# lzhangbj/deep_video_interpolation_extrapolation

Measured on AMD Instinct MI355X. Metric: train frames/s (256x512 len-3 clips), higher is better.
Workload: dtype bf16; 1 GPU; InterNet int_5_len_3 train step 256x512 bf16; per_gpu_batch=8, global_batch=8, parallelism=dp1, step=eager, executor side-stream lanes

## Files before the change

deep_video_interpolation_extrapolation_amd/_lib.py:

```python
import ctypes
import os
import threading

import torch

LIB_PATH = os.path.join(os.path.dirname(os.path.abspath(__file__)), "libdvie.so")

DVIE_OK = 0
DVIE_EINVAL = 1001
F32, BF16 = 0, 1
ACT_NONE, ACT_LRELU, ACT_ELU, ACT_RELU, ACT_TANH = 0, 1, 2, 3, 4
EW_FUSE, EW_UPT, EW_POOL, EW_POOLT, EW_COPY, EW_L1SIGN, EW_NCHW, EW_TONCHW, EW_MASK, EW_IM2COL, EW_LABELS = range(11)
LOSS_L1, LOSS_GDL, LOSS_SSIM, LOSS_MSE, LOSS_CE, LOSS_L1NHWC, LOSS_COSNHWC, LOSS_IOU, LOSS_ARGMAX_IOU = range(9)
OP_CONV, OP_WGRAD, OP_WREDUCE, OP_COLSUM, OP_EW, OP_LOSS, OP_PACK = 1, 2, 3, 4, 5, 6, 7
OP_BN_FWD, OP_BN_BWD, OP_HEAD_FWD, OP_HEAD_BWD, OP_ATTN, OP_HEAD3_BWD, OP_SEGENC_FWD = 8, 9, 10, 11, 12, 13, 14
OP_SEGENC_BWD = 15
OP_WREDUCE_MULTI = 16
OP_COSFEAT = 17
COSFEAT_MAX_TAPS = 8
YUV_420, YUV_444 = 420, 444
(ATTN_L2NORM, ATTN_L2NORM_BWD, ATTN_CORR, ATTN_GATHER, ATTN_GATHER_T, ATTN_SOFTMAX, ATTN_SOFTMAX_BWD, ATTN_WNORM,
 ATTN_WNORM_BWD, ATTN_POOL, ATTN_POOL_T) = range(11)

vp = ctypes.c_void_p
# ... 283 lines not shown
        ("n", i32), ("h", i32), ("w", i32), ("kpad0", i32), ("kpad2", i32), ("kpad4", i32),
    ]


class SegencBwdDesc(ctypes.Structure):
    _fields_ = [
        ("dout", vp), ("e2", vp), ("e1", vp), ("inp", vp), ("w4d", vp), ("w2d", vp),
        ("dw4", vp), ("dw2", vp), ("dw0", vp), ("db4", vp), ("db2", vp), ("db0", vp),
        ("dout_ld", i64), ("e2_ld", i64), ("e1_ld", i64), ("in_ld", i64),
        ("n", i32), ("h", i32), ("w", i32), ("kpad4", i32), ("kpad2", i32), ("slabs", i32),
    ]


class WreduceMultiDesc(ctypes.Structure):
    _fields_ = [("descs", vp), ("n", i32), ("pad", i32)]


class _OpUnion(ctypes.Union):
    _fields_ = [
        ("conv", ConvDesc), ("wgrad", WgradDesc), ("wreduce", WreduceDesc), ("colsum", ColsumDesc),
        ("ew", EwDesc), ("loss", LossDesc), ("pack", PackList), ("bn", BnDesc), ("head", HeadDesc),
        ("attn", AttnDesc), ("head3", Head3BwdDesc), ("segenc", SegencDesc), ("segenc_bwd", SegencBwdDesc),
        ("wreduce_multi", WreduceMultiDesc), ("cosfeat", CosFeatDesc),
    ]


class Op(ctypes.Structure):
    _fields_ = [("kind", i32), ("lane", i32), ("u", _OpUnion)]


_ABI = {0: Op, OP_CONV: ConvDesc, OP_WGRAD: WgradDesc, OP_WREDUCE: WreduceDesc, OP_COLSUM: ColsumDesc,
        OP_EW: EwDesc, OP_LOSS: LossDesc, OP_PACK: PackDesc, OP_BN_FWD: BnDesc, OP_HEAD_FWD: HeadDesc,
        OP_ATTN: AttnDesc, OP_HEAD3_BWD: Head3BwdDesc, OP_SEGENC_FWD: SegencDesc, OP_SEGENC_BWD: SegencBwdDesc, OP_WREDUCE_MULTI: WreduceMultiDesc,
        OP_COSFEAT: CosFeatDesc, 100: WarpDesc, 101: SoftmaxDesc, 102: SnLayer, 103: ClipDesc,
        104: SynthLoadDesc, 105: SynthFinishDesc, 106: SynthBridgeDesc, 107: SynthScoreDesc,
        108: SynthLoadPadDesc, 109: SynthFinishCropDesc, 110: SynthVggLoadDesc}
_ABI_MORE = {111: SynthMsssimDesc, 112: SynthYuvDesc, 113: SynthSceneDesc, 114: SynthCutFillDesc,
             115: SynthTileBlendDesc, 117: SynthRetimeDesc}

EXPORTS = [
    "dvie_conv2d_fwd", "dvie_conv2d_wgrad", "dvie_wgrad_splits_hint", "dvie_wgrad_slabs", "dvie_wgrad_reduce", "dvie_wgrad_reduce_multi", "dvie_colsum", "dvie_pack_weights",
    "dvie_ew", "dvie_loss", "dvie_loss_partial_count", "dvie_loss_ws_floats", "dvie_warp_fwd",
    "dvie_warp_bwd", "dvie_adamax", "dvie_scale", "dvie_run_ops", "dvie_abi_sizeof", "dvie_version",
    "dvie_last_error", "dvie_bn_fwd", "dvie_bn_bwd", "dvie_bn_partial_splits", "dvie_head_fwd", "dvie_head_bwd",
    "dvie_softmax_fwd", "dvie_softmax_bwd", "dvie_adam", "dvie_sn_fwd", "dvie_sn_bwd", "dvie_reparam_fwd",
    "dvie_reparam_bwd", "dvie_warp_ws_floats", "dvie_clip_prep", "dvie_attn", "dvie_step_inc", "dvie_adamax_dev",
    "dvie_adam_dev", "dvie_mfma_probe", "dvie_launch_probe", "dvie_sum_f32", "dvie_wgrad_bias_slabs", "dvie_head3_bwd",
    "dvie_segenc_fwd", "dvie_segenc_bwd", "dvie_pack_blocks", "dvie_trace_kernels", "dvie_traced_kernels",
    "dvie_synth_load", "dvie_synth_finish", "dvie_synth_bridge", "dvie_synth_score", "dvie_synth_score_ws_bytes",
    "dvie_synth_load_pad", "dvie_synth_finish_crop", "dvie_conv_zbits", "dvie_bn_partial_doubles",
    "dvie_synth_vgg_load", "dvie_cosfeat", "dvie_cosfeat_blocks", "dvie_synth_msssim", "dvie_synth_msssim_ws_bytes",
    "dvie_synth_yuv2rgb", "dvie_synth_rgb2yuv", "dvie_conv_chain", "dvie_conv2d_chain", "dvie_ops_chain_pairs",
    "dvie_synth_scene", "dvie_synth_scene_ws_bytes", "dvie_synth_cutfill", "dvie_synth_tile_blend",
    "dvie_synth_retime",
]

_lib = None
_lock = threading.Lock()


class DvieError(RuntimeError):
    pass


def load():
    global _lib
    if _lib is not None:
        return _lib
    with _lock:
        if _lib is not None:
            return _lib
        if not os.path.exists(LIB_PATH):
            raise DvieError(
                f"{LIB_PATH} is missing: build it with `python -c 'import __graft_entry__ as g; g.build()'` "
                "(there is no non-HIP fallback)")
        lib = ctypes.CDLL(LIB_PATH)
        lib.dvie_abi_sizeof.restype = ctypes.c_size_t
        lib.dvie_abi_sizeof.argtypes = [i32]
        for which, st in {**_ABI, **_ABI_MORE}.items():
            got = lib.dvie_abi_sizeof(which)
            if got != ctypes.sizeof(st):
                raise DvieError(f"ABI mismatch for {st.__name__}: C {got} vs ctypes {ctypes.sizeof(st)}")
        lib.dvie_version.restype = ctypes.c_char_p
        lib.dvie_last_error.restype = ctypes.c_char_p
        for name in ("dvie_conv2d_fwd", "dvie_conv2d_wgrad", "dvie_wgrad_reduce", "dvie_colsum", "dvie_ew",
                     "dvie_loss", "dvie_warp_fwd", "dvie_warp_bwd", "dvie_bn_fwd", "dvie_bn_bwd", "dvie_head_fwd",
                     "dvie_head_bwd", "dvie_softmax_fwd", "dvie_softmax_bwd", "dvie_clip_prep", "dvie_attn",
                     "dvie_head3_bwd", "dvie_segenc_fwd", "dvie_segenc_bwd", "dvie_synth_load", "dvie_synth_finish",
                     "dvie_synth_bridge", "dvie_synth_score", "dvie_synth_load_pad", "dvie_synth_finish_crop",
                     "dvie_synth_vgg_load", "dvie_cosfeat", "dvie_synth_msssim", "dvie_synth_yuv2rgb",
                     "dvie_synth_rgb2yuv", "dvie_synth_scene", "dvie_synth_cutfill", "dvie_synth_tile_blend",
                     "dvie_synth_retime"):
            getattr(lib, name).argtypes = [vp, vp]
            getattr(lib, name).restype = i32
        lib.dvie_pack_weights.argtypes = [vp, i32, i32, vp]
        lib.dvie_wgrad_reduce_multi.argtypes = [vp, i32, vp]
        lib.dvie_wgrad_reduce_multi.restype = i32
        lib.dvie_trace_kernels.argtypes = [i32]
        lib.dvie_trace_kernels.restype = i32
        lib.dvie_traced_kernels.argtypes = []
        lib.dvie_traced_kernels.restype = ctypes.c_char_p
        for name in ("dvie_wgrad_splits_hint", "dvie_wgrad_slabs", "dvie_bn_partial_splits", "dvie_pack_blocks",
                     "dvie_conv_zbits", "dvie_cosfeat_blocks"):
            getattr(lib, name).argtypes = [vp]
            getattr(lib, name).restype = i32
        lib.dvie_run_ops.argtypes = [vp, i32, vp]
        lib.dvie_conv_chain.argtypes = [vp, vp]
        lib.dvie_conv_chain.restype = i32
        lib.dvie_conv2d_chain.argtypes = [vp, vp, vp]
        lib.dvie_conv2d_chain.restype = i32
        lib.dvie_ops_chain_pairs.argtypes = [vp, i32, vp]
        lib.dvie_ops_chain_pairs.restype = i32
        lib.dvie_loss_partial_count.argtypes = [vp]
        lib.dvie_loss_partial_count.restype = ctypes.c_size_t
        lib.dvie_warp_ws_floats.argtypes = [vp]
        lib.dvie_warp_ws_floats.restype = ctypes.c_size_t
        lib.dvie_loss_ws_floats.argtypes = [vp]
        lib.dvie_loss_ws_floats.restype = ctypes.c_size_t
        lib.dvie_bn_partial_doubles.argtypes = [vp]
        lib.dvie_bn_partial_doubles.restype = ctypes.c_size_t
        lib.dvie_synth_score_ws_bytes.argtypes = [vp]
        lib.dvie_synth_score_ws_bytes.restype = ctypes.c_size_t
        lib.dvie_synth_msssim_ws_bytes.argtypes = [vp]
        lib.dvie_synth_msssim_ws_bytes.restype = ctypes.c_size_t
        lib.dvie_synth_scene_ws_bytes.argtypes = [vp]
        lib.dvie_synth_scene_ws_bytes.restype = ctypes.c_size_t
        lib.dvie_adamax.argtypes = [vp, vp, vp, vp, i64, f32, f32, f32, f32, f32, vp]
        lib.dvie_scale.argtypes = [vp, i64, f32, vp]
        lib.dvie_adam.argtypes = [vp, vp, vp, vp, i64, f32, f32, f32, f32, f32, vp]
        f64 = ctypes.c_double
        lib.dvie_adamax_dev.argtypes = [vp, vp, vp, vp, i64, f64, f64, f64, f64, f64, vp, vp]
        lib.dvie_adam_dev.argtypes = [vp, vp, vp, vp, i64, f64, f64, f64, f64, f64, vp, vp]
        lib.dvie_step_inc.argtypes = [vp, vp]
        lib.dvie_mfma_probe.argtypes = [vp, i32, i32, vp]
        lib.dvie_mfma_probe.restype = i32
        lib.dvie_launch_probe.argtypes = [i32, i32, vp]
        lib.dvie_launch_probe.restype = i32
        lib.dvie_sum_f32.argtypes = [vp, i32, vp, vp]
        lib.dvie_sum_f32.restype = i32
        lib.dvie_wgrad_bias_slabs.argtypes = [vp]
        lib.dvie_wgrad_bias_slabs.restype = i32
        for name in ("dvie_sn_fwd", "dvie_sn_bwd"):
            getattr(lib, name).argtypes = [vp, i32, vp, vp]
            getattr(lib, name).restype = i32
        lib.dvie_reparam_fwd.argtypes = [vp, vp, vp, vp, i64, vp]
        lib.dvie_reparam_bwd.argtypes = [vp, vp, vp, vp, vp, i64, i32, vp]
        lib.dvie_reparam_fwd.restype = lib.dvie_reparam_bwd.restype = i32
        _lib = lib
        return lib


def check(rc, what=""):
    if rc != DVIE_OK:
        msg = load().dvie_last_error().decode(errors="replace") if rc == DVIE_EINVAL else f"hipError {rc}"
        raise DvieError(f"{what}: {msg}")


def stream_ptr(device=None):
    return torch.cuda.current_stream(device).cuda_stream


def require_gpu(t):
    if not t.is_cuda:
        raise DvieError("dvie ops run on the MI355X only: tensor is on %s (no CPU fallback)" % t.device)
```

deep_video_interpolation_extrapolation_amd/csrc/segenc.hip:

```cpp
#include <stdlib.h>

#include <algorithm>
#include <type_traits>

#include "common.h"


namespace dvie {

typedef __attribute__((address_space(3))) void* lds_ptr_se;

struct SeCfg {
  static constexpr int NW = 8, R = 4, TW = 64;
  static constexpr int IN_W = TW + 6, IN_H = R + 6, IN_PITCH = 48;
  static constexpr int E1_W = TW + 4, E1_H = R + 4, E_PITCH = 80;
  static constexpr int E2_W = TW + 2, E2_H = R + 2;
  static constexpr int IN_SZ = IN_H * IN_W * IN_PITCH;
  static constexpr int IN_PC = (IN_SZ / 16 + 63) / 64;
  static constexpr int E1_SZ = E1_H * E1_W * E_PITCH;
  static constexpr int E2_SZ = E2_H * E2_W * E_PITCH;
  static constexpr int KS0 = 14, KS2 = 18;
  static constexpr int W0_PITCH = KS0 * 32 + 16, W2_PITCH = KS2 * 32 + 16;
  static constexpr int W0_SZ = 32 * W0_PITCH, W2_SZ = 32 * W2_PITCH, W4_SZ = 8 * W2_PITCH;
  static constexpr int O_W0 = 0, O_W2 = W0_SZ, O_W4 = O_W2 + W2_SZ, O_IN = O_W4 + W4_SZ;
// ... 152 lines not shown
          const bool in = (unsigned)gy < (unsigned)p.h && (unsigned)gx < (unsigned)p.w;
          const bool interior = r >= 2 && r < 2 + C::R && c >= 2 && c < 2 + C::TW && in;
#pragma unroll
          for (int P = 0; P < 2; ++P) {
            const int co = 16 * P + 8 * hh;
            i32x4 o;
#pragma unroll
            for (int e = 0; e < 4; ++e) {
              const float a = in ? elu_bf(v[P][2 * e] + bb0[P][2 * e]) : 0.f;
              const float b = in ? elu_bf(v[P][2 * e + 1] + bb0[P][2 * e + 1]) : 0.f;
              o[e] = (int)pack_bf16x2(a, b);
            }
            *(i32x4*)(smem + C::O_E1 + (r * C::E1_W + c) * C::E_PITCH + co * 2) = o;
            if (interior) *(i32x4*)((bf16_t*)p.e1 + ((long long)(n * p.h + gy) * p.w + gx) * p.e1_ld + co) = o;
          }
        });
    __syncthreads();
    se_stage<C::KS2, 4, C::E2_W, C::E_PITCH, C::W2_PITCH>(
        smem + C::O_W2, 32, smem + C::O_E1, C::E2_H * C::E2_W, wave, lane, [&](int r, int c, float (*v)[8]) {
          const int gy = y0 - 1 + r, gx = x0 - 1 + c;
          const bool in = (unsigned)gy < (unsigned)p.h && (unsigned)gx < (unsigned)p.w;
          const bool interior = r >= 1 && r < 1 + C::R && c >= 1 && c < 1 + C::TW && in;
#pragma unroll
          for (int P = 0; P < 2; ++P) {
            const int co = 16 * P + 8 * hh;
            i32x4 o;
#pragma unroll
            for (int e = 0; e < 4; ++e) {
              const float a = in ? elu_bf(v[P][2 * e] + bb2[P][2 * e]) : 0.f;
              const float b = in ? elu_bf(v[P][2 * e + 1] + bb2[P][2 * e + 1]) : 0.f;
              o[e] = (int)pack_bf16x2(a, b);
            }
            *(i32x4*)(smem + C::O_E2 + (r * C::E2_W + c) * C::E_PITCH + co * 2) = o;
            if (interior) *(i32x4*)((bf16_t*)p.e2 + ((long long)(n * p.h + gy) * p.w + gx) * p.e2_ld + co) = o;
          }
        });
    __syncthreads();
    se_stage<C::KS2, 4, C::TW, C::E_PITCH, C::W2_PITCH>(
        smem + C::O_W4, 8, smem + C::O_E2, C::R * C::TW, wave, lane, [&](int r, int c, float (*v)[8]) {
          const int gy = y0 + r, gx = x0 + c;
          if (hh || gy >= p.h || gx >= p.w) return;
          i32x4 o;
#pragma unroll
          for (int e = 0; e < 4; ++e) o[e] = (int)pack_bf16x2(v[0][2 * e] + bb4[2 * e], v[0][2 * e + 1] + bb4[2 * e + 1]);
          *(i32x4*)((bf16_t*)p.out + ((long long)(n * p.h + gy) * p.w + gx) * p.out_ld) = o;
        });
  }
}

}

extern "C" int dvie_segenc_fwd(const dvie_segenc_desc* d, void* stream) {
  using namespace dvie;
  DVIE_CHECK_ARG(d && d->in && d->e1 && d->e2 && d->out && d->w0 && d->w2 && d->w4, "segenc: null pointer");
  DVIE_CHECK_ARG(d->b0 && d->b2 && d->b4, "segenc: biases required");
  DVIE_CHECK_ARG(d->n > 0 && d->h > 0 && d->w > 0, "segenc: shape");
  DVIE_CHECK_ARG(d->in_ld >= 24 && d->e1_ld >= 32 && d->e2_ld >= 32 && d->out_ld >= 8, "segenc: leading dims");
  DVIE_CHECK_ARG(d->kpad0 >= 224 && d->kpad2 >= 288 && d->kpad4 >= 288, "segenc: kpad");
  const unsigned long long npx = (unsigned long long)d->n * d->h * d->w;
  DVIE_CHECK_ARG(npx * (unsigned long long)d->in_ld * 2ull < 0xFFFFFF00ull && npx < (1ull << 31),
                 "segenc: input exceeds the 32-bit buffer range");
  const int tiles_x = (d->w + 63) / 64, tiles_y = (d->h + 3) / 4;
  const long long nt = (long long)tiles_x * tiles_y * d->n;
  DVIE_CHECK_ARG(nt < (1LL << 30), "segenc: too many tiles");
  const int grid = (int)(nt < 256 ? nt : 256);
  DVIE_LAUNCH(segenc_fwd_kernel, dim3(grid), dim3(512), 0, (hipStream_t)stream, *d, tiles_x, tiles_y, (int)nt);
  DVIE_RETURN_LAUNCH();
}

namespace dvie {

__device__ __forceinline__ bf16x8 hb_tr_pair_se(const char* p0, const char* p1) {
  const s16x4 a = __builtin_amdgcn_ds_read_tr16_b64_v4i16((s16x4 __attribute__((address_space(3)))*)p0);
  const s16x4 b = __builtin_amdgcn_ds_read_tr16_b64_v4i16((s16x4 __attribute__((address_space(3)))*)p1);
  typedef short s16x8 __attribute__((ext_vector_type(8)));
  const s16x8 v = {a[0], a[1], a[2], a[3], b[0], b[1], b[2], b[3]};
  return __builtin_bit_cast(bf16x8, v);
}

__device__ __forceinline__ float sum8_bf16_se(const bf16x8 v, float t) {
  const i32x4 u = __builtin_bit_cast(i32x4, v);
  const bf16x2 one = __builtin_bit_cast(bf16x2, 0x3F803F80);
#pragma unroll
  for (int e = 0; e < 4; ++e) {
    const int w = u[e];
    t = __builtin_amdgcn_fdot2_f32_bf16(__builtin_bit_cast(bf16x2, w), one, t, false);
  }
  return t;
}

struct SbCfg {
  static constexpr int NW = 8, R = 4, TW = 64;
  static constexpr int DO_W = TW + 4, DO_H = R + 4;
  static constexpr int E_W = TW + 2, E_H = R + 2;
  static constexpr int DO_PC = (DO_H * DO_W + 63) / 64;
  static constexpr int E_PC = (E_H * E_W * 4 + 63) / 64;
  static constexpr int IN_PC = (E_H * E_W * 3 + 63) / 64;
  static constexpr int W4_PITCH = 5 * 32 + 16, W2_PITCH = 18 * 32 + 16;
  static constexpr int O_DO = 0, O_E2 = O_DO + DO_PC * 1024, O_E1 = O_E2 + E_PC * 1024, O_IN = O_E1 + E_PC * 1024;
  static constexpr int O_D2 = O_IN + IN_PC * 1024, O_D1 = O_D2 + E_H * E_W * 64, O_W4 = O_D1 + R * TW * 64;
  static constexpr int O_W2 = O_W4 + 32 * W4_PITCH, O_END = O_W2 + 32 * W2_PITCH;
  static constexpr int SMEM = O_END;
  static constexpr int PCS = DO_PC + 2 * E_PC + IN_PC;
  static constexpr int PQ = (PCS + NW - 1) / NW;
};
static_assert(SbCfg::SMEM <= 163840, "segenc backward LDS");
// ... 368 lines not shown
```

deep_video_interpolation_extrapolation_amd/csrc/warp_optim.hip:

```cpp
#include <stdlib.h>

#include <algorithm>
#include <vector>

#include "common.h"

namespace dvie {

__device__ __forceinline__ float linspace_pm1(int i, int n) {
  if (n <= 1) return -1.f;
  const float step = 2.f / (float)(n - 1);
  return (i < n / 2) ? __builtin_fmaf(step, (float)i, -1.f) : __builtin_fmaf(-step, (float)(n - 1 - i), 1.f);
}

__device__ __forceinline__ float unnorm(float g, int size, int ac) {
  return ac ? ((g + 1.f) / 2.f) * (float)(size - 1) : ((g + 1.f) * (float)size - 1.f) / 2.f;
}

struct WarpTap {
  int x0, y0;
  float ix, iy, wnw, wne, wsw, wse;
  bool vx0, vx1, vy0, vy1;
};

// ... 585 lines not shown
    case DVIE_OP_WREDUCE: reduce(o.u.wreduce); return true;
    case DVIE_OP_WREDUCE_MULTI:
      for (int k = 0; k < o.u.wreduce_multi.n; ++k) reduce(o.u.wreduce_multi.descs[k]);
      return true;
    case DVIE_OP_COLSUM: {
      const dvie_colsum_desc& d = o.u.colsum;
      const unsigned long long es = d.dtype == DVIE_BF16 ? 2 : 4;
      v.push_back({d.g, (unsigned long long)(d.rows - 1) * d.g_ld * es + d.c * es});
      v.push_back({d.ws, (unsigned long long)d.splits * d.c * 4ull});
      return true;
    }
    default: return false;
  }
}

extern "C" {

int dvie_ops_chain_pairs(const dvie_op* ops, int n, int* partner) {
  int pairs = 0;
  for (int i = 0; i < n; ++i) partner[i] = -1;
  if (!chain_on()) return 0;
  std::vector<OpSpan> sp;
  for (int i = 0; i + 1 < n; ++i) {
    if (partner[i] >= 0 || ops[i].kind != DVIE_OP_CONV || ops[i].lane != 0) continue;
    int j = i + 1;
    while (j < n && ops[j].lane == 1) ++j;
    if (j >= n || ops[j].kind != DVIE_OP_CONV || ops[j].lane != 0) continue;
    const dvie_conv_desc& a = ops[i].u.conv;
    const dvie_conv_desc& b = ops[j].u.conv;
    if (!dvie_conv_chain(&a, &b)) continue;
    const uintptr_t y0 = (uintptr_t)b.y;
    const unsigned long long yb = ((unsigned long long)b.n * b.yh * b.yw - 1) * b.y_ld * 2ull + b.cout * 2ull;
    bool ok = true;
    sp.clear();
    for (int k = i + 1; k < j && ok; ++k) ok = weight_op_spans(ops[k], sp);
    for (size_t k = 0; k < sp.size() && ok; ++k)
      if (sp[k].p && sp[k].bytes && (uintptr_t)sp[k].p < y0 + yb && y0 < (uintptr_t)sp[k].p + sp[k].bytes) ok = false;
    if (!ok) continue;
    partner[i] = j;
    partner[j] = i;
    ++pairs;
  }
  return pairs;
}

int dvie_run_ops(const dvie_op* ops, int n, void* stream) {
  LaneRun lr;
  lr.main = (hipStream_t)stream;
  std::vector<int> partner;
  if (n > 1 && chain_on()) {
    partner.resize(n);
    if (dvie_ops_chain_pairs(ops, n, partner.data()) == 0) partner.clear();
  }
  hipStreamCaptureStatus cap = hipStreamCaptureStatusNone;
  const bool capturing = hipStreamIsCapturing(lr.main, &cap) == hipSuccess && cap != hipStreamCaptureStatusNone;
  const bool lanes = lanes_on() && !capturing;
  auto finish = [&](int rc) {
    if (lr.d) {
      const hipError_t e = lr.finish();
      if (rc == DVIE_OK && e != hipSuccess) {
        set_error("run_ops: lane join failed");
        return (int)e;
      }
    }
    return rc;
  };
  for (int i = 0; i < n; ++i) {
    int rc = DVIE_OK;
    const dvie_op& o = ops[i];
    if (o.lane < 0 || o.lane > 1) {
      set_error("run_ops: lane %d of op %d out of range", o.lane, i);
      return finish(DVIE_EINVAL);
    }
    hipStream_t st = lr.main;
    if (lanes && o.lane == 1) {
      if (!lr.d) lr.d = lanes_of_device();
      if (!lr.d) {
        set_error("run_ops: side stream unavailable");
        return finish(DVIE_EINVAL);
      }
      if (lr.enter_weight() != hipSuccess) {
        set_error("run_ops: weight-lane wait failed at op %d", i);
        return finish(DVIE_EINVAL);
      }
      st = lr.d->side;
    } else {
      lr.tail_fresh = false;
    }
    void* s = (void*)st;
#ifdef DVIE_TIMING_DBG
    static const long long skip_kinds = getenv("DVIE_SKIP_KINDS") ? atoll(getenv("DVIE_SKIP_KINDS")) : 0;
    if ((skip_kinds >> o.kind) & 1) continue;
#endif
    if (!partner.empty() && partner[i] >= 0) {
      if (partner[i] < i) continue;
      rc = dvie_conv2d_chain(&o.u.conv, &ops[partner[i]].u.conv, s);
    } else
    switch (o.kind) {
      case DVIE_OP_CONV: rc = dvie_conv2d_fwd(&o.u.conv, s); break;
      case DVIE_OP_WGRAD: rc = dvie_conv2d_wgrad(&o.u.wgrad, s); break;
      case DVIE_OP_WREDUCE: rc = dvie_wgrad_reduce(&o.u.wreduce, s); break;
      case DVIE_OP_WREDUCE_MULTI: rc = dvie_wgrad_reduce_multi(o.u.wreduce_multi.descs, o.u.wreduce_multi.n, s); break;
      case DVIE_OP_COLSUM: rc = dvie_colsum(&o.u.colsum, s); break;
      case DVIE_OP_EW: rc = dvie_ew(&o.u.ew, s); break;
      case DVIE_OP_LOSS: rc = dvie_loss(&o.u.loss, s); break;
      case DVIE_OP_PACK: rc = dvie_pack_weights(o.u.pack.descs_dev, o.u.pack.n, o.u.pack.blocks, s); break;
      case DVIE_OP_BN_FWD: rc = dvie_bn_fwd(&o.u.bn, s); break;
      case DVIE_OP_BN_BWD: rc = dvie_bn_bwd(&o.u.bn, s); break;
      case DVIE_OP_HEAD_FWD: rc = dvie_head_fwd(&o.u.head, s); break;
      case DVIE_OP_HEAD_BWD: rc = dvie_head_bwd(&o.u.head, s); break;
      case DVIE_OP_ATTN: rc = dvie_attn(&o.u.attn, s); break;
      case DVIE_OP_HEAD3_BWD: rc = dvie_head3_bwd(&o.u.head3, s); break;
      case DVIE_OP_SEGENC_FWD: rc = dvie_segenc_fwd(&o.u.segenc, s); break;
      case DVIE_OP_SEGENC_BWD: rc = dvie_segenc_bwd(&o.u.segenc_bwd, s); break;
      case DVIE_OP_COSFEAT: rc = dvie_cosfeat(&o.u.cosfeat, s); break;
      default: set_error("run_ops: unknown op kind %d at %d", o.kind, i); return finish(DVIE_EINVAL);
    }
    if (rc != DVIE_OK) {
      if (rc == DVIE_EINVAL) {
        char buf[512];
        snprintf(buf, sizeof(buf), "op %d (kind %d): %s", i, o.kind, dvie_last_error());
        set_error("%s", buf);
      }
      return finish(rc);
    }
  }
  return finish(DVIE_OK);
}

size_t dvie_abi_sizeof(int which) {
  switch (which) {
    case 0: return sizeof(dvie_op);
    case DVIE_OP_CONV: return sizeof(dvie_conv_desc);
    case DVIE_OP_WGRAD: return sizeof(dvie_wgrad_desc);
    case DVIE_OP_WREDUCE: return sizeof(dvie_wreduce_desc);
    case DVIE_OP_WREDUCE_MULTI: return sizeof(dvie_wreduce_multi_desc);
    case DVIE_OP_COLSUM: return sizeof(dvie_colsum_desc);
    case DVIE_OP_EW: return sizeof(dvie_ew_desc);
    case DVIE_OP_LOSS: return sizeof(dvie_loss_desc);
    case DVIE_OP_PACK: return sizeof(dvie_pack_desc);
    case DVIE_OP_BN_FWD: return sizeof(dvie_bn_desc);
    case DVIE_OP_HEAD_FWD: return sizeof(dvie_head_desc);
    case DVIE_OP_ATTN: return sizeof(dvie_attn_desc);
    case DVIE_OP_HEAD3_BWD: return sizeof(dvie_head3_bwd_desc);
    case DVIE_OP_SEGENC_FWD: return sizeof(dvie_segenc_desc);
    case DVIE_OP_SEGENC_BWD: return sizeof(dvie_segenc_bwd_desc);
    case DVIE_OP_COSFEAT: return sizeof(dvie_cosfeat_desc);
// ... 25 lines not shown
```

include/dvie.h:

```cpp
#ifndef DVIE_H
#define DVIE_H

#include <stddef.h>
#include <stdint.h>

#ifdef __cplusplus
extern "C" {
#endif

#define DVIE_OK 0
#define DVIE_EINVAL 1001

#define DVIE_F32 0
#define DVIE_BF16 1

#define DVIE_ACT_NONE 0
#define DVIE_ACT_LRELU 1
#define DVIE_ACT_ELU 2
#define DVIE_ACT_RELU 3
#define DVIE_ACT_TANH 4

typedef struct dvie_conv_desc {
  const void* x;
  const void* w;
// ... 270 lines not shown
#define DVIE_ATTN_POOL 9
#define DVIE_ATTN_POOL_T 10

typedef struct dvie_attn_desc {
  const void* a;
  const void* b0;
  const void* b1;
  void* y;
  const void* res;
  const void* z;
  long long a_ld, b_ld, y_ld, res_ld, z_ld;
  int op, n, h, w;
  int c, wh, ww, nhalf;
  int half0, act, dact, beta;
  int dtype, pad0;
  float alpha, pad1;
} dvie_attn_desc;

int dvie_attn(const dvie_attn_desc* d, void* stream);

typedef struct dvie_head3_bwd_desc {
  const void* g;
  const void* h;
  const void* wd;
  void* dh;
  float* ws;
  long long g_ld, h_ld, dh_ld;
  int n, hgt, wid, c;
  int cout, kpad, dy0, dx0;
  int splits, dact;
  float alpha, pad0;
} dvie_head3_bwd_desc;

int dvie_head3_bwd(const dvie_head3_bwd_desc* d, void* stream);

typedef struct dvie_segenc_desc {
  const void* in;
  void* e1;
  void* e2;
  void* out;
  const void* w0;
  const void* w2;
  const void* w4;
  const float* b0;
  const float* b2;
  const float* b4;
  long long in_ld, e1_ld, e2_ld, out_ld;
  int n, h, w, kpad0;
  int kpad2, kpad4;
} dvie_segenc_desc;

int dvie_segenc_fwd(const dvie_segenc_desc* d, void* stream);

typedef struct dvie_segenc_bwd_desc {
  const void* dout;
  const void* e2;
  const void* e1;
  const void* in;
  const void* w4d;
  const void* w2d;
  float* dw4;
  float* dw2;
  float* dw0;
  float* db4;
  float* db2;
  float* db0;
  long long dout_ld, e2_ld, e1_ld, in_ld;
  int n, h, w, kpad4;
  int kpad2, slabs;
} dvie_segenc_bwd_desc;

int dvie_segenc_bwd(const dvie_segenc_bwd_desc* d, void* stream);

#define DVIE_OP_CONV 1
#define DVIE_OP_WGRAD 2
#define DVIE_OP_WREDUCE 3
#define DVIE_OP_COLSUM 4
#define DVIE_OP_EW 5
#define DVIE_OP_LOSS 6
#define DVIE_OP_PACK 7
#define DVIE_OP_BN_FWD 8
#define DVIE_OP_BN_BWD 9
#define DVIE_OP_HEAD_FWD 10
#define DVIE_OP_HEAD_BWD 11
#define DVIE_OP_ATTN 12
#define DVIE_OP_HEAD3_BWD 13
#define DVIE_OP_SEGENC_FWD 14
#define DVIE_OP_SEGENC_BWD 15
#define DVIE_OP_WREDUCE_MULTI 16
#define DVIE_OP_COSFEAT 17

#define DVIE_COSFEAT_MAX_TAPS 8

typedef struct dvie_cosfeat_desc {
  const void* feat;
  double* ws;
  double* out;
  long long ld;
  int mode, dtype, n, h, w, c, tap, n_taps, ws_blocks, pad0;
  int blocks[DVIE_COSFEAT_MAX_TAPS];
  int px[DVIE_COSFEAT_MAX_TAPS];
} dvie_cosfeat_desc;

int dvie_cosfeat_blocks(const dvie_cosfeat_desc* d);
int dvie_cosfeat(const dvie_cosfeat_desc* d, void* stream);

// ... 156 lines not shown
  uint8_t* cut;
  void* ws;
  long long s0, s1;
  long long sad_min, hist_min;
  int n0, n1, h, w;
} dvie_synth_scene_desc;

size_t dvie_synth_scene_ws_bytes(const dvie_synth_scene_desc* d);
int dvie_synth_scene(const dvie_synth_scene_desc* d, void* stream);

typedef struct dvie_synth_cutfill_desc {
  uint8_t* slots;
  const uint8_t* cut;
  long long s0, s1;
  long long nbytes;
  int n0, n1, levels, pad0;
} dvie_synth_cutfill_desc;

int dvie_synth_cutfill(const dvie_synth_cutfill_desc* d, void* stream);

#define DVIE_TILE_MAX 32
typedef struct dvie_synth_tile_blend_desc {
  const float* rgb_tiles;
  const float* seg_tiles;
  float* rgb_out;
  uint8_t* frame;
  uint8_t* label;
  uint8_t* label_canvas;
  int n, th, tw, hp, wp, h, w;
  int rgb_ld, seg_ld, n_classes, overlap;
  int nty, ntx, pad0;
  int ys[DVIE_TILE_MAX], xs[DVIE_TILE_MAX];
} dvie_synth_tile_blend_desc;

int dvie_synth_tile_blend(const dvie_synth_tile_blend_desc* d, void* stream);

typedef struct dvie_synth_retime_desc {
  const uint8_t* slots;
  uint8_t* out;
  const int32_t* rows;
  const int32_t* rows_dev;
  const uint8_t* cut;
  long long slot_s0, slot_s1, out_s0, out_s1;
  long long nbytes;
  int n0, n_slots, n_rows, n_pairs, den, pad0;
} dvie_synth_retime_desc;

int dvie_synth_retime(const dvie_synth_retime_desc* d, void* stream);

int dvie_run_ops(const dvie_op* ops, int n, void* stream);

int dvie_ops_chain_pairs(const dvie_op* ops, int n, int* partner);

size_t dvie_abi_sizeof(int which);
const char* dvie_version(void);
const char* dvie_last_error(void);

int dvie_trace_kernels(int on);
const char* dvie_traced_kernels(void);

#ifdef __cplusplus
}
#endif

#endif
```

Baseline: 264.2 frames/s.

## Add persistent segmentation-encoder forward kernel with prefetch and paired-map launches

Result: no change. 264.8 frames/s, median of 6 (+0.2%).

```diff
diff --git a/deep_video_interpolation_extrapolation_amd/_lib.py b/deep_video_interpolation_extrapolation_amd/_lib.py
--- a/deep_video_interpolation_extrapolation_amd/_lib.py
+++ b/deep_video_interpolation_extrapolation_amd/_lib.py
@@ -359,7 +359,8 @@
     "dvie_synth_vgg_load", "dvie_cosfeat", "dvie_cosfeat_blocks", "dvie_synth_msssim", "dvie_synth_msssim_ws_bytes",
     "dvie_synth_yuv2rgb", "dvie_synth_rgb2yuv", "dvie_conv_chain", "dvie_conv2d_chain", "dvie_ops_chain_pairs",
     "dvie_synth_scene", "dvie_synth_scene_ws_bytes", "dvie_synth_cutfill", "dvie_synth_tile_blend",
-    "dvie_synth_retime",
+    "dvie_synth_retime", "dvie_segenc_fwd2", "dvie_segenc_merge", "dvie_segenc2_on", "dvie_ops_segenc_pairs",
+    "dvie_segenc_lds_addr", "dvie_segenc_lds_info",
 ]
 
 _lib = None
@@ -418,6 +419,18 @@
         lib.dvie_conv2d_chain.restype = i32
         lib.dvie_ops_chain_pairs.argtypes = [vp, i32, vp]
         lib.dvie_ops_chain_pairs.restype = i32
+        lib.dvie_ops_segenc_pairs.argtypes = [vp, i32, vp]
+        lib.dvie_ops_segenc_pairs.restype = i32
+        lib.dvie_segenc_fwd2.argtypes = [vp, vp, vp]
+        lib.dvie_segenc_fwd2.restype = i32
+        lib.dvie_segenc_merge.argtypes = [vp, vp]
+        lib.dvie_segenc_merge.restype = i32
+        lib.dvie_segenc2_on.argtypes = []
+        lib.dvie_segenc2_on.restype = i32
+        lib.dvie_segenc_lds_addr.argtypes = [i32, i32, i32, i32]
+        lib.dvie_segenc_lds_addr.restype = i32
+        lib.dvie_segenc_lds_info.argtypes = [i32]
+        lib.dvie_segenc_lds_info.restype = i32
         lib.dvie_loss_partial_count.argtypes = [vp]
         lib.dvie_loss_partial_count.restype = ctypes.c_size_t
         lib.dvie_warp_ws_floats.argtypes = [vp]
diff --git a/deep_video_interpolation_extrapolation_amd/csrc/segenc.hip b/deep_video_interpolation_extrapolation_amd/csrc/segenc.hip
--- a/deep_video_interpolation_extrapolation_amd/csrc/segenc.hip
+++ b/deep_video_interpolation_extrapolation_amd/csrc/segenc.hip
@@ -228,6 +228,7 @@
 
 extern "C" int dvie_segenc_fwd(const dvie_segenc_desc* d, void* stream) {
   using namespace dvie;
+  if (dvie_segenc2_on()) return dvie_segenc_fwd2(d, nullptr, stream);
   DVIE_CHECK_ARG(d && d->in && d->e1 && d->e2 && d->out && d->w0 && d->w2 && d->w4, "segenc: null pointer");
   DVIE_CHECK_ARG(d->b0 && d->b2 && d->b4, "segenc: biases required");
   DVIE_CHECK_ARG(d->n > 0 && d->h > 0 && d->w > 0, "segenc: shape");
diff --git a/deep_video_interpolation_extrapolation_amd/csrc/segenc2.hip b/deep_video_interpolation_extrapolation_amd/csrc/segenc2.hip
--- /dev/null
+++ b/deep_video_interpolation_extrapolation_amd/csrc/segenc2.hip
@@ -0,0 +1,383 @@
+#include <stdlib.h>
+
+#include <type_traits>
+
+#include "common.h"
+#include "segenc_lds.h"
+
+namespace dvie {
+
+__device__ __forceinline__ float elu_bf_flat(float v) {
+  const float pl = v * (1.f + v * (0.5f + v * (1.f / 6.f)));
+  const float ex = __expf(v) - 1.f;
+  const float t = v > -0.03125f ? pl : ex;
+  return v > 0.f ? v : t;
+}
+
+template <int ST, int IN_S, int E2_V, typename Mid, typename Epi>
+__device__ __forceinline__ void se2_stage(const char* smem, int wave, int lane, int dbg, Mid&& mid, Epi&& epi) {
+  constexpr se2::Stage G = se2::stage(ST, IN_S, E2_V);
+  constexpr int KS = G.KS, NBLK = se2::blocks(G);
+  static_assert(NBLK <= 3 * se2::NW, "blocks per wave");
+  const int r32 = lane & 31, hh = lane >> 5;
+  const char* Wa = smem + G.WOFF + (r32 < G.WROWS ? r32 : r32 & (G.WROWS - 1)) * G.WP + hh * 16;
+  auto bfrag = [&](int px0, int s) {
+    const int kc = 2 * s + hh;
+    return *(const i32x4*)(smem + se2::src_off(ST, px0 + se2::tap_shift(G, kc), se2::tap_chunk(G, kc)));
+  };
+  auto finish = [&](const f32x16& acc, int q) {
+    float v[2][8];
+#pragma unroll
+    for (int P = 0; P < 2; ++P)
+#pragma unroll
+      for (int e = 0; e < 4; ++e) {
+        const auto sw = __builtin_amdgcn_permlane32_swap(__float_as_uint(acc[8 * P + e]),
+                                                         __float_as_uint(acc[8 * P + 4 + e]), false, false);
+        v[P][e] = __uint_as_float(sw[0]);
+        v[P][4 + e] = __uint_as_float(sw[1]);
+      }
+    const int r = q / G.RW, c = q - r * G.RW;
+    if (q < G.NPX && c < G.VW) epi(r, c, v);
+  };
+  auto mfma = [&](int blk0, auto nbt, f32x16 (&acc)[2], int (&q)[2]) {
+    constexpr int NB = decltype(nbt)::value;
+    int px0[NB];
+#pragma unroll
+    for (int b = 0; b < NB; ++b) {
+      q[b] = (blk0 + se2::NW * b) * 32 + r32;
+      px0[b] = se2::src_px(G, q[b]);
+#pragma unroll
+      for (int e = 0; e < 16; ++e) acc[b][e] = 0.f;
+    }
+    if (dbg & 64) return;
+    i32x4 fa[2], fb[2][NB];
+    auto ld = [&](int s, int buf) {
+      fa[buf] = *(const i32x4*)(Wa + s * 32);
+#pragma unroll
+      for (int b = 0; b < NB; ++b) fb[buf][b] = bfrag(px0[b], s);
+    };
+    ld(0, 0);
+#pragma unroll
+    for (int s = 0; s < KS; ++s) {
+      if (s + 1 < KS) ld(s + 1, (s + 1) & 1);
+      __builtin_amdgcn_sched_barrier(0);
+#pragma unroll
+      for (int b = 0; b < NB; ++b)
+        acc[b] = __builtin_amdgcn_mfma_f32_32x32x16_bf16(__builtin_bit_cast(bf16x8, fa[s & 1]),
+                                                         __builtin_bit_cast(bf16x8, fb[s & 1][b]), acc[b], 0, 0, 0);
+      __builtin_amdgcn_sched_barrier(0);
+    }
+  };
+  f32x16 acc[2];
+  int q[2];
+  const bool two = wave + se2::NW < NBLK;
+  if (two)
+    mfma(wave, std::integral_constant<int, 2>(), acc, q);
+  else
+    mfma(wave, std::integral_constant<int, 1>(), acc, q);
+  mid();
+  finish(acc[0], q[0]);
+  if (two) finish(acc[1], q[1]);
+  if (NBLK > 2 * se2::NW && wave + 2 * se2::NW < NBLK) {
+    mfma(wave + 2 * se2::NW, std::integral_constant<int, 1>(), acc, q);
+    finish(acc[0], q[0]);
+  }
+}
+
+template <int IN_S, int E2_V>
+__global__ __launch_bounds__(512) void segenc_fwd_kernel_v2(const dvie_segenc_desc pa, const dvie_segenc_desc pb,
+                                                            int tiles_x, int tiles_y, int nt1, int n_tiles, int dbg) {
+  namespace C = se2;
+  constexpr int NW = C::NW;
+  dbg = DVIE_DBG(dbg);
+  __shared__ __attribute__((aligned(1024))) char smem[C::SMEM];
+  const int tid = threadIdx.x, lane = tid & 63;
+  const int wave = __builtin_amdgcn_readfirstlane(tid >> 6);
+  const int hh = lane >> 5;
+  const unsigned OOB = 0xFFFFFFF0u;
+  const dvie_segenc_desc& p = pa;
+
+  auto wload = [&](const bf16_t* w, int kpad, int rows, int chunks, int pitch, int off) {
+    for (int i = tid; i < rows * chunks; i += NW * 64) {
+      const int r = i / chunks, ch = i - r * chunks;
+      *(i32x4*)(smem + off + r * pitch + ch * 16) = *(const i32x4*)(w + (size_t)r * kpad + ch * 8);
+    }
+  };
+  wload((const bf16_t*)p.w0, p.kpad0, 32, 2 * C::KS0, C::W0_PITCH, C::O_W0);
+  wload((const bf16_t*)p.w2, p.kpad2, 32, 2 * C::KS2, C::W2_PITCH, C::O_W2);
+  wload((const bf16_t*)p.w4, p.kpad4, 8, 2 * C::KS2, C::W2_PITCH, C::O_W4);
+
+  constexpr int IQ = C::IN_PC / NW;
+  int igeo[IQ];
+#pragma unroll
+  for (int q = 0; q < IQ; ++q) {
+    const int slot = (wave + NW * q) * 64 + lane, px = slot / 3, ch = slot - 3 * px;
+    const int row = px / IN_S, col = px - row * IN_S;
+    igeo[q] = row < C::IN_H && col < C::IN_W ? (row << 16) | (col << 4) | ch : -1;
+  }
+  const unsigned long long npx = (unsigned long long)p.n * p.h * p.w;
+  const unsigned irow = (unsigned)p.in_ld * 2u;
+  const int in_bytes = (int)((npx - 1) * p.in_ld * 2ull + 48ull);
+
+  float bb0[2][8], bb2[2][8], bb4[8];
+#pragma unroll
+  for (int P = 0; P < 2; ++P)
+#pragma unroll
+    for (int e = 0; e < 8; ++e) {
+      bb0[P][e] = p.b0[16 * P + 8 * hh + e];
+      bb2[P][e] = p.b2[16 * P + 8 * hh + e];
+    }
+#pragma unroll
+  for (int e = 0; e < 8; ++e) bb4[e] = p.b4[e];
+#pragma unroll
+  for (int P = 0; P < 2; ++P)
+#pragma unroll
+    for (int e = 0; e < 8; ++e) {
+      asm volatile("" : "+v"(bb0[P][e]));
+      asm volatile("" : "+v"(bb2[P][e]));
+    }
+#pragma unroll
+  for (int e = 0; e < 8; ++e) asm volatile("" : "+v"(bb4[e]));
+
+  struct Tile {
+    int m, n, y0, x0;
+  };
+  auto tile_pos = [&](int t) {
+    Tile T;
+    T.m = t >= nt1;
+    int tt = t - (T.m ? nt1 : 0);
+    T.x0 = (tt % tiles_x) * C::TW;
+    tt /= tiles_x;
+    T.y0 = (tt % tiles_y) * C::R;
+    T.n = tt / tiles_y;
+    return T;
+  };
+  i32x4 stg[IQ];
+  auto load_tile = [&](int t) {
+    const Tile T = tile_pos(t);
+    const __amdgpu_buffer_rsrc_t rin =
+        __builtin_amdgcn_make_buffer_rsrc((void*)(T.m ? pb.in : pa.in), 0, in_bytes, 0x00020000);
+#pragma unroll
+    for (int q = 0; q < IQ; ++q) {
+      const int v = igeo[q];
+      const int iy = T.y0 - 3 + ((v >> 16) & 0xFF), ix = T.x0 - 3 + ((v >> 4) & 0xFFF);
+      const bool ok = v >= 0 && (unsigned)iy < (unsigned)p.h && (unsigned)ix < (unsigned)p.w;
+      const unsigned o = ok ? (unsigned)((T.n * p.h + iy) * p.w + ix) * irow + (unsigned)(v & 15) * 16u : OOB;
+      stg[q] = __builtin_bit_cast(i32x4, __builtin_amdgcn_raw_buffer_load_b128(rin, o, 0, 0));
+    }
+  };
+  auto store_tile = [&]() {
+#pragma unroll
+    for (int q = 0; q < IQ; ++q) *(i32x4*)(smem + C::in_store_addr(wave + NW * q, lane)) = stg[q];
+  };
+  const int G = gridDim.x;
+  int t = blockIdx.x;
+  if (t >= n_tiles) return;
+  load_tile(t);
+  store_tile();
+  if (t + G < n_tiles) load_tile(t + G);
+  __syncthreads();
+
+  for (; t < n_tiles; t += G) {
+    const Tile T = tile_pos(t);
+    const int n = T.n, y0 = T.y0, x0 = T.x0;
+    bf16_t* const ge1 = (bf16_t*)(T.m ? pb.e1 : pa.e1);
+    bf16_t* const ge2 = (bf16_t*)(T.m ? pb.e2 : pa.e2);
+    bf16_t* const gout = (bf16_t*)(T.m ? pb.out : pa.out);
+    auto elu_store = [&](int st, float (*v)[8], const float (*bb)[8], bool in, bool interior, int lp, bf16_t* gp) {
+#pragma unroll
+      for (int P = 0; P < 2; ++P) {
+        i32x4 o;
+#pragma unroll
+        for (int e = 0; e < 4; ++e) {
+          const float s0 = v[P][2 * e] + bb[P][2 * e], s1 = v[P][2 * e + 1] + bb[P][2 * e + 1];
+          const int pk = (int)((dbg & 32)  ? pack_bf16x2(s0, s1)
+                               : (dbg & 4) ? pack_bf16x2(elu_bf(s0), elu_bf(s1))
+                                           : pack_bf16x2(elu_bf_flat(s0), elu_bf_flat(s1)));
+          o[e] = in ? pk : 0;
+        }
+        *(i32x4*)(smem + (st == 0 ? C::e1_off(lp, 2 * P + hh) : C::e2_off(lp, 2 * P + hh))) = o;
+        if (interior && !(dbg & 16)) *(i32x4*)(gp + 16 * P + 8 * hh) = o;
+      }
+    };
+    se2_stage<0, IN_S, E2_V>(
+        smem, wave, lane, dbg, [] {},
+        [&](int r, int c, float (*v)[8]) {
+          const int gy = y0 - 2 + r, gx = x0 - 2 + c;
+          const bool in = (unsigned)gy < (unsigned)p.h && (unsigned)gx < (unsigned)p.w;
+          const bool interior = r >= 2 && r < 2 + C::R && c >= 2 && c < 2 + C::TW && in;
+          elu_store(0, v, bb0, in, interior, r * C::E1_S + c, ge1 + ((long long)(n * p.h + gy) * p.w + gx) * p.e1_ld);
+        });
+    __syncthreads();
+    se2_stage<1, IN_S, E2_V>(
+        smem, wave, lane, dbg,
+        [&] {
+          if (dbg & 128) return;
+          if (t + G < n_tiles) store_tile();
+          if (t + 2 * G < n_tiles) load_tile(t + 2 * G);
+        },
+        [&](int r, int c, float (*v)[8]) {
+          const int gy = y0 - 1 + r, gx = x0 - 1 + c;
+          const bool in = (unsigned)gy < (unsigned)p.h && (unsigned)gx < (unsigned)p.w;
+          const bool interior = r >= 1 && r < 1 + C::R && c >= 1 && c < 1 + C::TW && in;
+          elu_store(1, v, bb2, in, interior, r * C::E2_S + c, ge2 + ((long long)(n * p.h + gy) * p.w + gx) * p.e2_ld);
+        });
+    __syncthreads();
+    se2_stage<2, IN_S, E2_V>(
+        smem, wave, lane, dbg, [] {},
+        [&](int r, int c, float (*v)[8]) {
+          const int gy = y0 + r, gx = x0 + c;
+          if (hh || gy >= p.h || gx >= p.w || (dbg & 16)) return;
+          i32x4 o;
+#pragma unroll
+          for (int e = 0; e < 4; ++e) o[e] = (int)pack_bf16x2(v[0][2 * e] + bb4[2 * e], v[0][2 * e + 1] + bb4[2 * e + 1]);
+          *(i32x4*)(gout + ((long long)(n * p.h + gy) * p.w + gx) * p.out_ld) = o;
+        });
+  }
+}
+
+static const char* segenc_check(const dvie_segenc_desc* d) {
+  if (!(d && d->in && d->e1 && d->e2 && d->out && d->w0 && d->w2 && d->w4)) return "segenc: null pointer";
+  if (!(d->b0 && d->b2 && d->b4)) return "segenc: biases required";
+  if (!(d->n > 0 && d->h > 0 && d->w > 0)) return "segenc: shape";
+  if (!(d->in_ld >= 24 && d->e1_ld >= 32 && d->e2_ld >= 32 && d->out_ld >= 8)) return "segenc: leading dims";
+  if (!(d->kpad0 >= 224 && d->kpad2 >= 288 && d->kpad4 >= 288)) return "segenc: kpad";
+  const unsigned long long npx = (unsigned long long)d->n * d->h * d->w;
+  if (!(npx * (unsigned long long)d->in_ld * 2ull < 0xFFFFFF00ull && npx < (1ull << 31)))
+    return "segenc: input exceeds the 32-bit buffer range";
+  return nullptr;
+}
+
+struct SeSpan {
+  uintptr_t p;
+  unsigned long long bytes;
+};
+static SeSpan se_span(const void* p, unsigned long long npx, long long ld, int c) {
+  return {(uintptr_t)p, (npx - 1) * (unsigned long long)ld * 2ull + (unsigned long long)c * 2ull};
+}
+static bool se_overlap(const SeSpan& a, const SeSpan& b) { return a.p < b.p + b.bytes && b.p < a.p + a.bytes; }
+
+}
+
+using namespace dvie;
+
+extern "C" int dvie_segenc2_on(void) {
+  const char* e = getenv("DVIE_SEGENC2");
+  return !(e && *e == '0');
+}
+
+extern "C" int dvie_segenc_merge(const dvie_segenc_desc* a, const dvie_segenc_desc* b) {
+  if (segenc_check(a) || segenc_check(b)) return 0;
+  if (a->w0 != b->w0 || a->w2 != b->w2 || a->w4 != b->w4 || a->b0 != b->b0 || a->b2 != b->b2 || a->b4 != b->b4) return 0;
+  if (a->n != b->n || a->h != b->h || a->w != b->w) return 0;
+  if (a->kpad0 != b->kpad0 || a->kpad2 != b->kpad2 || a->kpad4 != b->kpad4) return 0;
+  if (a->in_ld != b->in_ld || a->e1_ld != b->e1_ld || a->e2_ld != b->e2_ld || a->out_ld != b->out_ld) return 0;
+  const unsigned long long npx = (unsigned long long)a->n * a->h * a->w;
+  const SeSpan wa[3] = {se_span(a->e1, npx, a->e1_ld, 32), se_span(a->e2, npx, a->e2_ld, 32), se_span(a->out, npx, a->out_ld, 8)};
+  const SeSpan wb[3] = {se_span(b->e1, npx, b->e1_ld, 32), se_span(b->e2, npx, b->e2_ld, 32), se_span(b->out, npx, b->out_ld, 8)};
+  const SeSpan ia = se_span(a->in, npx, a->in_ld, 24), ib = se_span(b->in, npx, b->in_ld, 24);
+  for (int i = 0; i < 3; ++i) {
+    if (se_overlap(wa[i], ib) || se_overlap(wb[i], ia)) return 0;
+    for (int j = 0; j < 3; ++j) {
+      if (!se_overlap(wa[i], wb[j])) continue;
+      const long long row = a->out_ld * 2, off = (long long)((uintptr_t)b->out - (uintptr_t)a->out);
+      const long long m = ((off % row) + row) % row;
+      if (!(i == 2 && j == 2 && m >= 16 && m <= row - 16 && (off >= 0 ? off : -off) < row)) return 0;
+    }
+  }
+  return 1;
+}
+
+static bool input_op_spans(const dvie_op& o, SeSpan& y, SeSpan (&rd)[2]) {
+  if (o.kind != DVIE_OP_EW || o.lane != 0) return false;
+  const dvie_ew_desc& d = o.u.ew;
+  if (d.op != DVIE_EW_NCHW && d.op != DVIE_EW_LABELS) return false;
+  if (d.res || d.z || d.beta || d.src0 || d.src2 || !d.y || d.n <= 0 || d.h <= 0 || d.w <= 0) return false;
+  const unsigned long long es = d.dtype == DVIE_BF16 ? 2 : 4, npx = (unsigned long long)d.n * d.h * d.w;
+  y = {(uintptr_t)d.y, (npx - 1) * (unsigned long long)d.y_ld * es + (unsigned long long)d.c * es};
+  if (d.sn < 0 || d.sc < 0 || d.sh < 0 || d.sw < 0) return false;
+  const unsigned long long ext_es = d.op == DVIE_EW_LABELS ? 1 : 4;
+  const unsigned long long last = (unsigned long long)(d.n - 1) * d.sn + (unsigned long long)(d.ext_c > 0 ? d.ext_c - 1 : 0) * d.sc +
+                                  (unsigned long long)(d.h - 1) * d.sh + (unsigned long long)(d.w - 1) * d.sw;
+  rd[0] = {(uintptr_t)d.ext, d.ext ? (last + 1) * ext_es : 0ull};
+  rd[1] = {(uintptr_t)d.src1, d.src1 ? (last + 1) * 4ull : 0ull};
+  return true;
+}
+
+extern "C" int dvie_ops_segenc_pairs(const dvie_op* ops, int n, int* partner) {
+  int pairs = 0;
+  for (int i = 0; i < n; ++i) partner[i] = -1;
+  if (!dvie_segenc2_on()) return 0;
+  for (int i = 0; i + 1 < n; ++i) {
+    if (partner[i] >= 0 || ops[i].kind != DVIE_OP_SEGENC_FWD || ops[i].lane != 0) continue;
+    const dvie_segenc_desc& a = ops[i].u.segenc;
+    if (segenc_check(&a)) continue;
+    const unsigned long long npx = (unsigned long long)a.n * a.h * a.w;
+    const SeSpan wr[3] = {se_span(a.e1, npx, a.e1_ld, 32), se_span(a.e2, npx, a.e2_ld, 32), se_span(a.out, npx, a.out_ld, 8)};
+    const SeSpan in = se_span(a.in, npx, a.in_ld, 24);
+    int j = i + 1;
+    bool ok = true;
+    for (; j < n && ok && ops[j].kind != DVIE_OP_SEGENC_FWD; ++j) {
+      SeSpan y, rd[2];
+      ok = input_op_spans(ops[j], y, rd) && !se_overlap(y, in);
+      for (int k = 0; k < 3 && ok; ++k)
+        ok = !se_overlap(y, wr[k]) && !(rd[0].bytes && se_overlap(rd[0], wr[k])) && !(rd[1].bytes && se_overlap(rd[1], wr[k]));
+    }
+    if (!ok || j >= n || ops[j].lane != 0 || !dvie_segenc_merge(&a, &ops[j].u.segenc)) continue;
+    partner[i] = j;
+    partner[j] = i;
+    ++pairs;
+  }
+  return pairs;
+}
+
+extern "C" int dvie_segenc_fwd2(const dvie_segenc_desc* a, const dvie_segenc_desc* b, void* stream) {
+  if (const char* msg = segenc_check(a)) DVIE_CHECK_ARG(false, "%s", msg);
+  DVIE_CHECK_ARG(!b || dvie_segenc_merge(a, b), "segenc: the two maps do not share one launch");
+  const int tiles_x = (a->w + 63) / 64, tiles_y = (a->h + 3) / 4;
+  const long long nt1 = (long long)tiles_x * tiles_y * a->n, nt = b ? 2 * nt1 : nt1;
+  DVIE_CHECK_ARG(nt < (1LL << 30), "segenc: too many tiles");
+  int grid = (int)(nt < 256 ? nt : 256);
+  int dbg = 0;
+  if (const char* e = getenv("DVIE_SEGENC2_GRID")) {
+    const int g = atoi(e);
+    if (g > 0 && g < grid) grid = g;
+  }
+#ifdef DVIE_TIMING_DBG
+  if (const char* e = getenv("DVIE_SEGENC2_DBG")) dbg = atoi(e);
+  if (dbg & 8) {
+    DVIE_LAUNCH((segenc_fwd_kernel_v2<70, 66>), dim3(grid), dim3(512), 0, (hipStream_t)stream, *a, b ? *b : *a, tiles_x,
+                tiles_y, (int)nt1, (int)nt, dbg);
+    DVIE_RETURN_LAUNCH();
+  }
+#endif
+  DVIE_LAUNCH((segenc_fwd_kernel_v2<se2::IN_S, se2::E2_V>), dim3(grid), dim3(512), 0, (hipStream_t)stream, *a,
+              b ? *b : *a, tiles_x, tiles_y, (int)nt1, (int)nt, dbg);
+  DVIE_RETURN_LAUNCH();
+}
+
+extern "C" int dvie_segenc_lds_addr(int pattern, int blk, int step, int lane) {
+  namespace C = se2;
+  if (lane < 0 || lane > 63 || blk < 0 || step < 0) return -2;
+  if (pattern >= 0 && pattern <= 2) {
+    const C::Stage g = C::stage(pattern);
+    return blk < C::blocks(g) && step < g.KS ? C::b_addr(pattern, blk, step, lane) : -2;
+  }
+  if (pattern >= 3 && pattern <= 5) return step < C::stage(pattern - 3).KS ? C::a_addr(pattern - 3, step, lane) : -2;
+  if (pattern == 6 || pattern == 7)
+    return blk < C::blocks(C::stage(pattern - 6)) && step < 2 ? C::w_addr(pattern - 6, blk, step, lane) : -2;
+  if (pattern == 8) return blk < C::IN_PC ? C::in_store_addr(blk, lane) : -2;
+  return -2;
+}
+
+extern "C" int dvie_segenc_lds_info(int what) {
+  namespace C = se2;
+  switch (what) {
+    case 0: return C::SMEM;
+    case 1: case 2: case 3: return C::blocks(C::stage(what - 1));
+    case 4: case 5: case 6: return C::stage(what - 4).KS;
+    case 7: return C::IN_PC;
+    case 8: return 2;
+    default: return -1;
+  }
+}
diff --git a/deep_video_interpolation_extrapolation_amd/csrc/segenc_lds.h b/deep_video_interpolation_extrapolation_amd/csrc/segenc_lds.h
--- /dev/null
+++ b/deep_video_interpolation_extrapolation_amd/csrc/segenc_lds.h
@@ -0,0 +1,67 @@
+#pragma once
+
+namespace dvie {
+namespace se2 {
+
+constexpr int NW = 8, R = 4, TW = 64;
+constexpr int KS0 = 14, KS2 = 18;
+constexpr int W0_PITCH = KS0 * 32 + 16, W2_PITCH = KS2 * 32 + 16;
+constexpr int IN_H = R + 6, IN_W = TW + 6, IN_S = 84, IN_PITCH = 48;
+constexpr int IN_PC = (IN_H * IN_S * 3 + 63) / 64;
+constexpr int E1_H = R + 4, E1_W = TW + 4, E1_S = E1_W, E1_PITCH = 80, E1_SLACK = 10;
+constexpr int E2_H = R + 2, E2_W = TW + 2, E2_V = E1_W, E2_S = E2_V, E2_PITCH = 64;
+constexpr int O_W0 = 0, O_W2 = O_W0 + 32 * W0_PITCH, O_W4 = O_W2 + 32 * W2_PITCH, O_IN = O_W4 + 8 * W2_PITCH;
+constexpr int O_E1 = O_IN + IN_PC * 1024, O_E2 = O_E1 + (E1_H * E1_S + E1_SLACK) * E1_PITCH;
+constexpr int SMEM = O_E2 + E2_H * E2_S * E2_PITCH;
+static_assert(IN_PC == NW * 5, "input DMA: five 1-KB pieces per wave");
+static_assert(SMEM <= 163840, "segenc forward LDS");
+
+struct Stage {
+  int RW, VW, NPX, S, CPT, KS, WP, WOFF, WROWS;
+};
+constexpr Stage stage(int st, int in_s = IN_S, int e2_v = E2_V) {
+  return st == 0   ? Stage{E1_W, E1_W, E1_H * E1_W, in_s, 3, KS0, W0_PITCH, O_W0, 32}
+         : st == 1 ? Stage{e2_v, E2_W, E2_H * e2_v, E1_S, 4, KS2, W2_PITCH, O_W2, 32}
+                   : Stage{TW, TW, R * TW, E2_S, 4, KS2, W2_PITCH, O_W4, 8};
+}
+constexpr int blocks(const Stage& g) { return (g.NPX + 31) / 32; }
+
+constexpr int e2_swz(int p) { return ((p >> 2) ^ (p & 2)) & 3; }
+constexpr int in_off(int p, int c) { return O_IN + p * IN_PITCH + c * 16; }
+constexpr int e1_off(int p, int c) { return O_E1 + p * E1_PITCH + c * 16; }
+constexpr int e2_off(int p, int c) { return O_E2 + p * E2_PITCH + ((c ^ e2_swz(p)) << 4); }
+constexpr int src_off(int st, int p, int c) { return st == 0 ? in_off(p, c) : st == 1 ? e1_off(p, c) : e2_off(p, c); }
+constexpr int dst_off(int st, int p, int c) { return st == 0 ? e1_off(p, c) : e2_off(p, c); }
+constexpr int dst_stride(int st) { return st == 0 ? E1_S : E2_S; }
+
+constexpr int src_px(const Stage& g, int q) { return (q / g.RW) * g.S + q % g.RW; }
+constexpr int tap_shift(const Stage& g, int kc) {
+  const int k = kc < 9 * g.CPT ? kc : 9 * g.CPT - 1, t = k / g.CPT;
+  return (t / 3) * g.S + t % 3;
+}
+constexpr int tap_chunk(const Stage& g, int kc) { return (kc < 9 * g.CPT ? kc : 9 * g.CPT - 1) % g.CPT; }
+
+constexpr int b_addr(int st, int blk, int s, int lane, int in_s = IN_S, int e2_v = E2_V) {
+  const Stage g = stage(st, in_s, e2_v);
+  const int kc = 2 * s + (lane >> 5);
+  return src_off(st, src_px(g, blk * 32 + (lane & 31)) + tap_shift(g, kc), tap_chunk(g, kc));
+}
+constexpr int a_addr(int st, int s, int lane) {
+  const Stage g = stage(st);
+  const int r = lane & 31;
+  return g.WOFF + (r < g.WROWS ? r : r & (g.WROWS - 1)) * g.WP + (lane >> 5) * 16 + s * 32;
+}
+constexpr int w_addr(int st, int blk, int P, int lane, int e2_v = E2_V) {
+  const Stage g = stage(st, IN_S, e2_v);
+  const int q = blk * 32 + (lane & 31), r = q / g.RW, c = q % g.RW;
+  return q < g.NPX && c < g.VW ? dst_off(st, r * dst_stride(st) + c, 2 * P + (lane >> 5)) : -1;
+}
+constexpr int in_store_addr(int pc, int lane) { return O_IN + pc * 1024 + lane * 16; }
+
+static_assert(src_px(stage(0), E1_H * E1_W - 1) + tap_shift(stage(0), 26) < IN_H * IN_S, "e1 stage reads");
+static_assert(src_px(stage(1), blocks(stage(1)) * 32 - 1) + tap_shift(stage(1), 35) < E1_H * E1_S + E1_SLACK,
+              "e2 stage reads");
+static_assert(src_px(stage(2), R * TW - 1) + tap_shift(stage(2), 35) < E2_H * E2_S, "out stage reads");
+
+}
+}
diff --git a/deep_video_interpolation_extrapolation_amd/csrc/warp_optim.hip b/deep_video_interpolation_extrapolation_amd/csrc/warp_optim.hip
--- a/deep_video_interpolation_extrapolation_amd/csrc/warp_optim.hip
+++ b/deep_video_interpolation_extrapolation_amd/csrc/warp_optim.hip
@@ -661,6 +661,11 @@
     partner.resize(n);
     if (dvie_ops_chain_pairs(ops, n, partner.data()) == 0) partner.clear();
   }
+  std::vector<int> seg;
+  if (n > 1 && dvie_segenc2_on()) {
+    seg.resize(n);
+    if (dvie_ops_segenc_pairs(ops, n, seg.data()) == 0) seg.clear();
+  }
   hipStreamCaptureStatus cap = hipStreamCaptureStatusNone;
   const bool capturing = hipStreamIsCapturing(lr.main, &cap) == hipSuccess && cap != hipStreamCaptureStatusNone;
   const bool lanes = lanes_on() && !capturing;
@@ -701,7 +706,10 @@
     static const long long skip_kinds = getenv("DVIE_SKIP_KINDS") ? atoll(getenv("DVIE_SKIP_KINDS")) : 0;
     if ((skip_kinds >> o.kind) & 1) continue;
 #endif
-    if (!partner.empty() && partner[i] >= 0) {
+    if (!seg.empty() && seg[i] >= 0) {
+      if (seg[i] > i) continue;
+      rc = dvie_segenc_fwd2(&ops[seg[i]].u.segenc, &o.u.segenc, s);
+    } else if (!partner.empty() && partner[i] >= 0) {
       if (partner[i] < i) continue;
       rc = dvie_conv2d_chain(&o.u.conv, &ops[partner[i]].u.conv, s);
     } else
diff --git a/include/dvie.h b/include/dvie.h
--- a/include/dvie.h
+++ b/include/dvie.h
@@ -346,6 +346,12 @@
 
 int dvie_segenc_fwd(const dvie_segenc_desc* d, void* stream);
 
+int dvie_segenc_fwd2(const dvie_segenc_desc* a, const dvie_segenc_desc* b, void* stream);
+int dvie_segenc_merge(const dvie_segenc_desc* a, const dvie_segenc_desc* b);
+int dvie_segenc2_on(void);
+int dvie_segenc_lds_addr(int pattern, int blk, int step, int lane);
+int dvie_segenc_lds_info(int what);
+
 typedef struct dvie_segenc_bwd_desc {
   const void* dout;
   const void* e2;
@@ -608,6 +614,8 @@
 
 int dvie_ops_chain_pairs(const dvie_op* ops, int n, int* partner);
 
+int dvie_ops_segenc_pairs(const dvie_op* ops, int n, int* partner);
+
 size_t dvie_abi_sizeof(int which);
 const char* dvie_version(void);
 const char* dvie_last_error(void);
```
